# Simencassiman/P2PMicrogrid

Measured on AMD Instinct MI355X. Metric: agent-steps/sec (whole node, rollout+Q-update) at 1/2/4/8 MI355X; % HBM roofline, higher is better.
Workload: dtype f32 simulation, f64 Q-table

## Files before the change

### p2pmicrogrid_amd/csrc/p2pmg_fast.hip

```cpp
#include "p2pmg_fastmath.h"

namespace p2pmg {
namespace {

template <typename QT>
__device__ __forceinline__ Row4<QT> fake_row(const QT* p) {
  const uint32_t x = (uint32_t)(reinterpret_cast<uintptr_t>(p) >> 5);
  return Row4<QT>{{(QT)(x & 3), (QT)((x >> 2) & 3), (QT)((x >> 4) & 3), (QT)0}};
}

template <int N, int D, int G>
__device__ __forceinline__ void gather_even(float ev, float (&col)[N], int i) {
  if constexpr (D < G) {
    const float got = shfl_xor_c<D>(ev);
    const int src = i ^ D;
#pragma unroll
    for (int k = 0; k < N; ++k) col[k] = (k == src) ? got : col[k];
    gather_even<N, D + 1, G>(ev, col, i);
  }
}

#ifndef P2PMG_BAT_SPEC
#define P2PMG_BAT_SPEC 1
#endif
template <int N, typename QT, int R1, bool TRAIN, int BAT, bool NARROW, bool PIPE = false>
__global__ __launch_bounds__(kWave) void episode_fast_kernel(const EpisodeParams p, const uint2* __restrict__ pre,
                                                             FastRec* __restrict__ recs, int spw, int n_cons,
                                                             const PrepOut nxt) {
  if ((int)blockIdx.x >= n_cons) {
    const size_t n = (size_t)p.T * p.A, stride = (size_t)(gridDim.x - n_cons) * kWave;
    const int n_ep = nxt.n_ep > 1 ? nxt.n_ep : 1;
    for (int ep = 0; ep < n_ep; ++ep)
      for (size_t k2 = (size_t)(blockIdx.x - n_cons) * kWave + threadIdx.x; k2 < n; k2 += stride)
        prepass_one(p, nxt, k2, ep);
    return;
  }
  constexpr int G = pow2ceil(N);
  static_assert(G <= 8 && R1 >= 1 && R1 <= 4, "fast path: G <= 8, R + 1 <= 4");
  static_assert(!PIPE || (TRAIN && BAT == 0), "two episodes per wave: chained training launches without a battery");
  constexpr bool CAND = N == 2 && R1 >= 2 && BAT == 0;
  const int lane = (int)threadIdx.x;
  const int grp = PIPE ? lane >> 5 : 0;
  const int hl = PIPE ? (lane & 31) : lane;
  const int sl = hl / G;
  const int i = hl % G;
  const int s = (int)blockIdx.x * spw + sl;
  const bool active = i < N && sl < spw && s < p.S;
  const int a = active ? s * N + i : 0;
  const int s_env = p.n_env == 1 ? 0 : (active ? s : 0);
  const int T = p.T;
  const size_t A = (size_t)p.A;
  const KC k = pin_constants(p, p.thermal[a]);
  const uint32_t n_states = (uint32_t)(p.nt * p.nT * p.nb * p.np);
  QT* __restrict__ q = reinterpret_cast<QT*>(p.q) + (size_t)a * n_states * kQPad;
  const int a_first = (int)blockIdx.x * spw * N;
  constexpr uint32_t kRowShift = sizeof(QT) == 8 ? 5 : 4;
  const char* const qwave = reinterpret_cast<const char*>(p.q) + ((size_t)a_first * n_states << kRowShift);
  const uint32_t qlane = active ? (uint32_t)(a - a_first) * (n_states << kRowShift) : 0u;
  auto gat = [&](uint32_t row) __attribute__((always_inline)) {
    return gather_row(reinterpret_cast<const QT*>(qwave + (qlane + (row << kRowShift))));
  };
  const int np = k.np;
  const int nbv = k.nb;
  const float km1_T = (float)(k.nT - 1), km2_T = (float)(k.nT - 2), km1_p = (float)(np - 1), kp = (float)np;
  const float mi = active ? p.max_in[a] : 1.0f;
  const Recip rmi = recip(mi), rmph = recip(k.mph), rn = recip((float)N);
  const float4 lv = p.hp_lv[a];
  const float hin[3] = {(k.c_in * lv.x) * k.cop, (k.c_in * lv.y) * k.cop, (k.c_in * lv.z) * k.cop};
  const float hm[3] = {(k.c_m * lv.x) * k.cop, (k.c_m * lv.y) * k.cop, (k.c_m * lv.z) * k.cop};
  float tin = active ? p.t_in[a] : k.setpoint;
  float tm = active ? p.t_m[a] : k.setpoint;
  double bcap = 0.0, soc = 0.0;
  BatK bk{};
  Recip64 rcap{};
  if constexpr (BAT != 0) {
    bcap = active ? p.bat_cap[a] : 0.0;
    soc = active ? p.soc[a] : 0.0;
    bk = BatK{p.bat_min, p.bat_max, p.bat_sqrt_eff, recip64_u(p.bat_sqrt_eff), kR900};
    rcap = recip64(bcap > 0.0 ? bcap : 1.0);
  }
  const int ip_zero = idx_plain(div_n<N>(0.0f) / mi, np);
  QT* const q_dummy = reinterpret_cast<QT*>(p.dummy) + lane * kQPad;
  constexpr bool narrow = NARROW;
  const size_t rec_bytes = narrow ? sizeof(float2) : sizeof(FastRec);
  char* const rec_dummy = reinterpret_cast<char*>(reinterpret_cast<FastRec*>(p.dummy) + kWave + lane);
  const bool rec_on = p.record != 0 && active;
  const size_t rec_step = rec_on ? A * rec_bytes : 0;

  auto temp_bin = [&](float t_in) {
    const float x = t_in - k.setpoint;
    return clamp_bin_f(((x + 1.0f) / 2.0f) * km2_T + 1.0f, km1_T);
  };
  auto p2p_bin = [&](float x) { return clamp_bin_f(((x + 1.0f) / 2.0f) * kp, km1_p); };

  const float* envb = p.env + (size_t)s_env * kEnvStride;
  const size_t env_step = (size_t)p.n_env * kEnvStride;
  const uint2* preb = pre + a;
  const uint32_t* ipc_a = p.pre_ipc + a;
  const int t1 = T > 1 ? 1 : 0, t2 = 2 % T;
  const int n_chain = p.chain > 1 ? p.chain : 1;
  bool st_on = active;
  size_t rec_adv = rec_step;
  bool wrap_l = false;
  bool wrap_it = false;
  QT* snap = nullptr;
  if constexpr (PIPE) {
    __shared__ QT snap_lds[2 * 32 * 32];
    snap = snap_lds;
  }
  const uint32_t* codes_a;
  char* rec_ptr;
  uint32_t TA, env_st, env_end, o3, eo3;
  EnvV eS[3];
  uint2 pS[3];
  uint32_t cS[3];
  uint32_t cw, strip, a0, aN;
  int iT;
  Row4<QT> row0, rowN;
  uint32_t iS[3] = {0u, 0u, 0u};
  Row4<QT> cand[3];
  Patch<QT> pat{0xFFFFFFFFu, 0, (QT)0};
  float ep_sum = 0.0f;
  float t0_in = tin, t0_m = tm;
  auto code_of = [&](uint32_t w) { return TRAIN ? w : 0xFFFFFFFFu; };
  auto strip_of = [&](uint32_t base, int it_) { return __umul24(base + __umul24((uint32_t)it_, (uint32_t)nbv), (uint32_t)np); };
  auto row0_addr = [&](uint32_t st, uint32_t nr, uint32_t c) -> uint32_t {
    const bool need = ((c & 0xFF) == 255) || (TRAIN && R1 == 1);
    return need ? st + (uint32_t)ip_zero : nr;
  };
#if P2PMG_TRACE
  uint64_t trW = 0, trC = 0, trR = 0, trLast = 0, trA0 = 0, trWC = 0, trA1 = 0, trMid = 0, trCal = 0;
#define P2PMG_STAMP(v) asm volatile("s_memtime %0\n s_waitcnt lgkmcnt(0)" : "=s"(v)::"memory")
#endif
  auto begin_episode = [&](int ep) __attribute__((always_inline)) {
    if constexpr (PIPE) {
      if (ep >= 1 && st_on) {
        tin = t0_in;
        tm = t0_m;
      }
    }
    codes_a = p.codes + (size_t)(PIPE && ep < 0 ? 0 : ep) * p.codes_stride + a;
    if constexpr (PIPE) {
      rec_ptr = rec_on && st_on ? reinterpret_cast<char*>(recs) + (size_t)a * rec_bytes : rec_dummy;
      rec_adv = st_on ? rec_step : 0;
    } else {
      rec_ptr = rec_on ? reinterpret_cast<char*>(recs) + (size_t)a * rec_bytes : rec_dummy;
    }
    TA = (uint32_t)T * (uint32_t)A, env_st = (uint32_t)env_step, env_end = env_st * (uint32_t)T;
    o3 = (uint32_t)(3 % T) * (uint32_t)A, eo3 = (uint32_t)(3 % T) * env_st;

    eS[0] = load_envv(envb), eS[1] = load_envv(envb + (size_t)t1 * env_step), eS[2] = load_envv(envb + (size_t)t2 * env_step);
    pS[0] = preb[0], pS[1] = preb[(size_t)t1 * A], pS[2] = preb[(size_t)t2 * A];
    cS[0] = codes_a[0], cS[1] = codes_a[(size_t)t1 * A], cS[2] = codes_a[(size_t)t2 * A];
    cw = code_of(cS[0]);
    iT = temp_bin(tin);
    strip = strip_of(pS[0].y & 0xFFFFu, iT);
    const uint32_t nrow = strip_of(pS[0].y >> 16, iT) + (uint32_t)ip_zero;
    a0 = row0_addr(strip, nrow, cw);
    aN = TRAIN ? nrow : a0;
    row0 = gat(a0);
    rowN = gat(aN);
    if constexpr (CAND) {
      iS[0] = ipc_a[0];
      iS[1] = ipc_a[(size_t)t1 * A];
      iS[2] = ipc_a[(size_t)t2 * A];
#pragma unroll
      for (int b = 0; b < 3; ++b) cand[b] = gat((strip + ((iS[0] >> (8 * b)) & 0xFFu)));
    }
    pat = Patch<QT>{0xFFFFFFFFu, 0, (QT)0};
    ep_sum = 0.0f;
    if constexpr (!PIPE) {
      t0_in = tin, t0_m = tm;
      if (p.reset_t0 && active)
        t0_draw(p.seed_lo, p.seed_hi, p.episode + ep + 1, p.agent_offset + (uint32_t)a, k.setpoint, p.reset_sigma, t0_in,
                t0_m);
    } else {
      constexpr int kSnap = 10;
      const uint32_t key0 = pS[0].y & 0xFFFFu;
      const int nTi = p.nT;
      Row4<QT> sr[kSnap];
      auto snap_load = [&](int it0) {
#pragma unroll
        for (int j = 0; j < kSnap; ++j) sr[j] = gat(strip_of(key0, it0 + j < nTi ? it0 + j : nTi - 1) + (uint32_t)ip_zero);
      };
      auto snap_store = [&](int it0) {
#pragma unroll
        for (int j = 0; j < kSnap; ++j)
          if (it0 + j < nTi) snap[(grp * 32 + it0 + j) * 32 + hl] = max3(sr[j]);
      };
      snap_load(0);
      if (active)
        t0_draw(p.seed_lo, p.seed_hi, p.episode + (ep + 2 < n_chain ? ep + 2 : n_chain), p.agent_offset + (uint32_t)a,
                k.setpoint, p.reset_sigma, t0_in, t0_m);
      snap_store(0);
      for (int it0 = kSnap; it0 < nTi; it0 += kSnap) {
        snap_load(it0);
        snap_store(it0);
      }
    }
  };
  auto end_episode = [&](int ep) __attribute__((always_inline)) {
    if (active) {
      if (p.reset_t0) {
        tin = t0_in;
        tm = t0_m;
      }
      if (i == 0) {
        if (p.chain_rewards) p.chain_rewards[(size_t)ep * p.S + s] = ep_sum;
        if (ep == n_chain - 1) p.ep_reward[s] = ep_sum;
      }
    }
  };

  auto step = [&](auto par) __attribute__((always_inline)) {
    constexpr int P = decltype(par)::value, P1 = (P + 1) % 3;
    const EnvV ev = eS[P];
    const EnvRow e0{0.0f, ev.x, ev.y, ev.z, ev.w};
    const uint2 p0 = pS[P], p1 = pS[P1];
    const uint32_t c1 = cS[P1], ipc0 = iS[P], ipc1 = iS[P1];
    const float balw = __uint_as_float(p0.x);
    float row[N];
    float col[N];
#pragma unroll
    for (int j = 0; j < N; ++j) { row[j] = 0.0f; col[j] = 0.0f; }
    float tinA[3];
    uint32_t iTA[3], stA[3], nrA[3];
    {
      const float ain = k.inv_ri * (tm - tin) + k.inv_rvent * (e0.t_out - tin);
#pragma unroll
      for (int x = 0; x < 3; ++x) {
        const float d_in = k.inv_ci * (ain + hin[x]);
        tinA[x] = tin + (d_in * k.spm) * k.slot;
        iTA[x] = (uint32_t)temp_bin(tinA[x]);
        stA[x] = strip_of(p1.y & 0xFFFFu, (int)iTA[x]);
        nrA[x] = strip_of(p1.y >> 16, (int)iTA[x]) + (uint32_t)ip_zero;
      }
    }
    const Patch<QT> pprev = pat;
#if P2PMG_TRACE
    uint64_t tr0, tr1;
    P2PMG_STAMP(tr0);
    if (trLast) trR += tr0 - trLast;
    asm volatile("" ::"v"(row0.v[0]), "v"(row0.v[1]), "v"(row0.v[2]));
    P2PMG_STAMP(tr1);
    trW += tr1 - tr0;
    {
      uint64_t tcal;
      P2PMG_STAMP(tcal);
      trCal += tcal - tr1;
      tr1 = tcal;
    }
    trMid = tr1;
#endif
    double soc_r = soc;
    BatPre bpre{};
    if constexpr (BAT == 2) bpre = bat_pre(soc, bcap, bk);
    auto bat_rule = [&](float o, double& sr) -> float {
      if constexpr (BAT == 2) return (float)battery_rule_pre((double)o, sr, rcap, bk, bpre);
      return (float)battery_rule_r<true>((double)o, sr, bcap, rcap, bk);
    };
    row0 = patched(row0, a0, pat);

    int code = (int)(cw & 0xFF);
    int act = code == 255 ? argmax3(row0) : code;
    float hp = hp_of(lv, act);
    int ip = ip_zero;
    Row4<QT> rowR = row0;
    uint32_t acts = (uint32_t)act, ips = (uint32_t)ip_zero;
    float tin1 = tin, tm1 = tm;
    int iT1 = 0;
    uint32_t strip1 = 0, cw1 = 0, a0n = 0, aNn = 0;
    Row4<QT> row0n, rowNn, candn[3];
    Sel3M mnext{};
    auto issue_next = [&](int act_final) {
      const Sel3M m = sel3_masks(act_final);
// ... 117 lines not shown
        trC += trLast - trMid;
#endif
        refill_words();
        settle_next();
      }
      float out = balw + hp;
      if constexpr (BAT != 0) {
#if P2PMG_BAT_SPEC
        if (r == R1 - 1) {
          const Sel3M m = sel3_masks(act);
          out = sel3(m, outA[0], outA[1], outA[2]);
          soc_r = sel3(m, socA[0], socA[1], socA[2]);
        } else
#endif
        {
          soc_r = soc;
          if (bcap > 0.0) out = bat_rule(out, soc_r);
        }
      }
#if P2PMG_ABLATE == 11
      if (r == R1 - 1) {
        row[0] = out;
        continue;
      }
#endif
      const float flo = out < 0.0f ? 0.0f : -__builtin_inff(), fhi = out > 0.0f ? 0.0f : __builtin_inff();
      float f[N];
      float tot = 0.0f;
#pragma unroll
      for (int j = 0; j < N; ++j) {
        const float pw = -((j == i) ? 0.0f : col[j]);
        f[j] = __builtin_amdgcn_fmed3f(pw, flo, fhi);
        tot = tot + f[j];
      }
      tot = fabsf(tot);
      const float ev = div_n_r<N>(out * 1.0f, rn);
      const Recip rt = recip(tot == 0.0f ? 1.0f : tot);
      const float nout = nabs_out(out);
      float num[N];
      bool bad = !rt.ok;
#pragma unroll
      for (int j = 0; j < N; ++j) {
        num[j] = nout * f[j];
        row[j] = fdiv_core(num[j], rt);
        bad = bad || !fdiv_ok(num[j]);
      }
      if (bad) {
#pragma unroll
        for (int j = 0; j < N; ++j) row[j] = fdiv_ieee(num[j], rt.b);
      }
#pragma unroll
      for (int j = 0; j < N; ++j) row[j] = (tot == 0.0f) ? ev : row[j];
    }
    soc = soc_r;
    pat.row = 0xFFFFFFFFu;

    float g = 0.0f, pp = 0.0f;
#if P2PMG_ABLATE == 11
    g = row[0];
#else
    exchange<N>(row, col, i, sl, nullptr);
#pragma unroll
    for (int j = 0; j < N; ++j) {
      const float pij = row[j], pji = col[j];
      const float ex = pair_exchange(pij, pji);
      g = g + (pij - ex);
      pp = pp + ex;
    }
#endif
    float cost = (g >= 0.0f) ? g * e0.buy : g * e0.inj;
    cost = cost + pp * e0.p2p;
    cost = fdiv_b(cost * k.slot, rmph);
    cost = cost * k.kilo;
    float pen = fmaxf(fmaxf(0.0f, k.lower - tin), fmaxf(0.0f, tin - k.upper));
    pen = pen > 0.0f ? pen + 1.0f : 0.0f;
    const float rw = -(cost + k.penw * pen);

    if constexpr (TRAIN) {
      const uint32_t srow = strip + (uint32_t)ip;
      const QT qsa = sel3(act, rowR.v[0], rowR.v[1], rowR.v[2]);
      QT qmax = max3(patched(rowN, aN, pprev));
      if constexpr (PIPE && P == 2) {
        if (wrap_it) {
          const QT sv = snap[((grp ^ 1) * 32 + iT) * 32 + hl];
#if P2PMG_ABLATE != 12
          qmax = wrap_l ? sv : qmax;
#endif
        }
      }
      const QT qnew = td_update(qsa, rw, qmax, k.alpha, k.gamma);
      *((PIPE ? st_on : active) ? q + srow * kQPad + act : q_dummy) = qnew;
#if P2PMG_ABLATE == 9 || P2PMG_ABLATE == 10
      pat = Patch<QT>{0xFFFFFFFFu, 0, (QT)0};
#else
      pat = Patch<QT>{srow, act, qnew};
#endif
    }
    if constexpr (narrow) {
      *reinterpret_cast<float2*>(__builtin_assume_aligned(rec_ptr, 8)) = make_float2(rw, cost);
    } else {
      const uint32_t bins = (p0.y & 0xFFFFu) | ((uint32_t)iT << 16);
      float4* rp = reinterpret_cast<float4*>(__builtin_assume_aligned(rec_ptr, 16));
      rp[0] = make_float4(rw, cost, g, pp);
      rp[1] = make_float4(tin, __uint_as_float(acts), __uint_as_float(bins), __uint_as_float(ips));
    }
    rec_ptr += PIPE ? rec_adv : rec_step;
    asm volatile("" ::: "memory");
    eS[P] = load_envv(envb + eo3);
    pS[P] = preb[o3];
    const float m = group_sum<N>(rw, lane, i, sl, nullptr);
    ep_sum = ep_sum + div_n_r<N>(m, rn);

    tin = tin1;
    tm = tm1;
    iT = iT1;
    o3 += (uint32_t)A;
    o3 = o3 == TA ? 0u : o3;
    eo3 += env_st;
    eo3 = eo3 == env_end ? 0u : eo3;
    strip = strip1;
    cw = cw1;
    a0 = a0n;
    aN = aNn;
    row0 = row0n;
    rowN = rowNn;
    if constexpr (CAND) {
#pragma unroll
      for (int b = 0; b < 3; ++b) cand[b] = candn[b];
    }
  };
  using S0 = std::integral_constant<int, 0>;
  using S1 = std::integral_constant<int, 1>;
  using S2 = std::integral_constant<int, 2>;
  if constexpr (!PIPE) {
    for (int ep = 0; ep < n_chain; ++ep) {
      begin_episode(ep);
      __builtin_amdgcn_s_waitcnt(0);
      int t = 0;
      for (; t + 3 <= T; t += 3) {
        step(S0{});
        step(S1{});
        step(S2{});
      }
      if (t < T) step(S0{});
      if (t + 1 < T) step(S1{});
#if P2PMG_TRACE
      if (threadIdx.x == 0 && (blockIdx.x == 0 || (int)blockIdx.x == n_cons / 2 || (int)blockIdx.x == n_cons - 1))
        printf("TRACE blk %d/%d T %d: per step wait %.1f round0 %.1f waitcand %.1f round1 %.1f issue %.1f rest %.1f "
               "(one stamp %.1f)\n",
               (int)blockIdx.x, n_cons, T, (double)trW / T, (double)trA0 / T, (double)trWC / T, (double)trA1 / T,
               (double)trC / T, (double)trR / (T - 1), (double)trCal / T);
      trW = trC = trR = trLast = trA0 = trWC = trA1 = trMid = trCal = 0;
#endif
      end_episode(ep);
    }
    if (active) {
      p.t_in[a] = tin;
      p.t_m[a] = tm;
      if constexpr (BAT != 0) p.soc[a] = soc;
    }
  } else {
    const int L = T / 2;
    int ep_l = grp == 0 ? 0 : -1;
    st_on = active && grp == 0;
    begin_episode(ep_l);
    __builtin_amdgcn_s_waitcnt(0);
    for (int ph = 0;; ++ph) {
      if (ph > 0) {
        if (grp == (ph & 1)) {
          if (st_on && i == 0) {
            if (p.chain_rewards) p.chain_rewards[(size_t)ep_l * p.S + s] = ep_sum;
            if (ep_l == n_chain - 1) p.ep_reward[s] = ep_sum;
          }
          if (ph <= n_chain) {
            ep_l = ph;
            st_on = active && ph < n_chain;
            begin_episode(ph < n_chain ? ph : n_chain - 1);
          }
        }
        __builtin_amdgcn_s_waitcnt(0);
        if (ph > n_chain) break;
      }
      wrap_l = st_on && grp != (ph & 1) && ep_l + 1 < n_chain;
      for (int t = 0; t < L; t += 3) {
        wrap_it = t + 3 >= L;
        step(S0{});
        step(S1{});
        step(S2{});
      }
    }
    if (active && grp == ((n_chain - 1) & 1)) {
      p.t_in[a] = t0_in;
      p.t_m[a] = t0_m;
    }
  }
}

template <int N>
constexpr bool kFastPipe = N == 2;

template <int N, typename QT, int R1, int BAT, bool NARROW>
void launch_fast_nw(const EpisodeParams& p, const uint2* pre, FastRec* recs, int blocks, int spw, int prod,
                    const PrepOut& nxt, hipEvent_t ev0, hipEvent_t ev1, hipStream_t st) {
  if constexpr (kFastPipe<N> && BAT == 0) {
    if (p.mode == 0 && p.interleave)
      return hipExtLaunchKernelGGL((episode_fast_kernel<N, QT, R1, true, BAT, NARROW, true>), dim3(blocks + prod),
                                   dim3(kWave), 0, st, ev0, ev1, 0, p, pre, recs, spw, blocks, nxt);
  }
  if (p.mode == 0)
    hipExtLaunchKernelGGL((episode_fast_kernel<N, QT, R1, true, BAT, NARROW>), dim3(blocks + prod), dim3(kWave), 0, st,
                          ev0, ev1, 0, p, pre, recs, spw, blocks, nxt);
  else
    hipExtLaunchKernelGGL((episode_fast_kernel<N, QT, R1, false, BAT, NARROW>), dim3(blocks + prod), dim3(kWave), 0, st,
                          ev0, ev1, 0, p, pre, recs, spw, blocks, nxt);
}
template <int N, typename QT, int R1, int BAT>
void launch_fast_b(const EpisodeParams& p, const uint2* pre, FastRec* recs, int blocks, int spw, int prod,
                   const PrepOut& nxt, hipEvent_t ev0, hipEvent_t ev1, hipStream_t st) {
  if (p.rec_narrow) return launch_fast_nw<N, QT, R1, BAT, true>(p, pre, recs, blocks, spw, prod, nxt, ev0, ev1, st);
  launch_fast_nw<N, QT, R1, BAT, false>(p, pre, recs, blocks, spw, prod, nxt, ev0, ev1, st);
}
template <int N, typename QT, int R1>
void launch_fast_r(const EpisodeParams& p, const uint2* pre, FastRec* recs, int blocks, int spw, int prod,
                   const PrepOut& nxt, hipEvent_t ev0, hipEvent_t ev1, hipStream_t st) {
  if constexpr (R1 <= kFastBatMaxR1) {
    if (p.battery && p.bat_safe) return launch_fast_b<N, QT, R1, 2>(p, pre, recs, blocks, spw, prod, nxt, ev0, ev1, st);
    if (p.battery) return launch_fast_b<N, QT, R1, 1>(p, pre, recs, blocks, spw, prod, nxt, ev0, ev1, st);
  }
  launch_fast_b<N, QT, R1, 0>(p, pre, recs, blocks, spw, prod, nxt, ev0, ev1, st);
}

template <int N, typename QT>
hipError_t launch_fast_n(const EpisodeParams& p, const uint2* pre, void* recs, int spw, const PrepOut* nxt,
                         hipEvent_t ev0, hipEvent_t ev1, hipStream_t st) {
  constexpr int G = pow2ceil(N);
  if (p.interleave && !(kFastPipe<N> && p.mode == 0 && !p.battery && p.chain >= 2 && p.reset_t0 && p.T % 6 == 0 &&
                        p.nT <= 32 && spw > 0 && spw <= kWave / 2 / G))
    return hipErrorInvalidValue;
  if (spw <= 0 || spw > kWave / G) spw = kWave / G;
  const int blocks = (p.S + spw - 1) / spw;
  const size_t n = (size_t)p.T * p.A;
  const int prod = nxt ? (int)std::min<size_t>(2048, (n + kWave - 1) / kWave) : 0;
  const PrepOut none{nullptr, nullptr, nullptr, 0, 0.0};
  FastRec* r = reinterpret_cast<FastRec*>(recs);
  switch (p.R + 1) {
    case 1: launch_fast_r<N, QT, 1>(p, pre, r, blocks, spw, prod, nxt ? *nxt : none, ev0, ev1, st); break;
    case 2: launch_fast_r<N, QT, 2>(p, pre, r, blocks, spw, prod, nxt ? *nxt : none, ev0, ev1, st); break;
    case 3: launch_fast_r<N, QT, 3>(p, pre, r, blocks, spw, prod, nxt ? *nxt : none, ev0, ev1, st); break;
    case 4: launch_fast_r<N, QT, 4>(p, pre, r, blocks, spw, prod, nxt ? *nxt : none, ev0, ev1, st); break;
    default: return hipErrorInvalidValue;
  }
  return hipGetLastError();
}

template <int N0>
hipError_t launch_fast_pair(const EpisodeParams& p, const uint2* pre, void* recs, int q_dtype, int spw,
                            const PrepOut* nxt, hipEvent_t ev0, hipEvent_t ev1, hipStream_t st) {
  if (p.N == N0)
    return q_dtype == 0 ? launch_fast_n<N0, double>(p, pre, recs, spw, nxt, ev0, ev1, st)
                        : launch_fast_n<N0, float>(p, pre, recs, spw, nxt, ev0, ev1, st);
  if (p.N == N0 + 1)
    return q_dtype == 0 ? launch_fast_n<N0 + 1, double>(p, pre, recs, spw, nxt, ev0, ev1, st)
                        : launch_fast_n<N0 + 1, float>(p, pre, recs, spw, nxt, ev0, ev1, st);
  return hipErrorInvalidValue;
}

}

#define P2PMG_FAST_LAUNCHER(name, N0)                                                                             \
  hipError_t name(const EpisodeParams& p, const uint2* pre, void* recs, int q_dtype, int spw, const PrepOut* next, \
                  hipEvent_t ev0, hipEvent_t ev1, hipStream_t stream) {                                           \
    return launch_fast_pair<N0>(p, pre, recs, q_dtype, spw, next, ev0, ev1, stream);                              \
  }
#if P2PMG_FAST_SLICE == 0
P2PMG_FAST_LAUNCHER(launch_fast_n12, 1)
#endif
#if P2PMG_FAST_SLICE == 1
P2PMG_FAST_LAUNCHER(launch_fast_n34, 3)
#endif
#if P2PMG_FAST_SLICE == 2
P2PMG_FAST_LAUNCHER(launch_fast_n56, 5)
#endif
#if P2PMG_FAST_SLICE == 3
P2PMG_FAST_LAUNCHER(launch_fast_n78, 7)
#endif
#if P2PMG_FAST_SLICE == 0
hipError_t launch_episode_fast(const EpisodeParams& p, const uint2* pre, void* recs, int q_dtype, int spw,
                               const PrepOut* next, hipEvent_t ev0, hipEvent_t ev1, hipStream_t stream) {
  auto f = p.N <= 2 ? launch_fast_n12 : p.N <= 4 ? launch_fast_n34 : p.N <= 6 ? launch_fast_n56 : launch_fast_n78;
  if (p.N < 1 || p.N > 8) return hipErrorInvalidValue;
  return f(p, pre, recs, q_dtype, spw, next, ev0, ev1, stream);
}
#endif

}
```

### p2pmicrogrid_amd/csrc/p2pmg_plan.cpp

```cpp
#include "p2pmg_plan.h"

#include <algorithm>
#include <cmath>

#include "p2pmg_internal.h"

namespace p2pmg {
namespace {

bool host_div_range(float b) {
  const float m = std::fabs(b);
  return m >= 0x1p-40f && m <= 0x1p40f;
}

bool fast_applies(const PlanFacts& c, const p2pmg_episode_args& args, const Overrides& ov) {
  const p2pmg_config& g = c.cfg;
  return !g.shared_q && (!c.battery || c.R + 1 <= kFastBatMaxR1) && c.N <= 8 && c.R + 1 <= 4 && c.mi_ok &&
         (long long)g.n_time_states * g.n_temp_states * g.n_balance_states < 65536 &&
         64LL * g.n_time_states * g.n_temp_states * g.n_balance_states * g.n_p2p_states * 4 * (g.q_dtype == 0 ? 8 : 4) <
             (1LL << 32) &&
         (long long)c.T * c.A < (1LL << 32) && host_div_range(g.minutes_per_hour) &&
         g.temp_margin == 1.0f &&
         !(args.flags & (P2PMG_FLAG_GENERAL_KERNEL | P2PMG_FLAG_TILE_KERNEL | P2PMG_FLAG_PHILOX_INKERNEL)) &&
         !ov.general;
}

}

EpisodePlan plan_episode(const PlanFacts& c, const p2pmg_episode_args& args, bool chained, const Overrides& ov,
                         int n_chain) {
  const p2pmg_config& g = c.cfg;
  const bool train = args.mode == P2PMG_MODE_TRAIN;
  const bool philox = train && args.rng == P2PMG_RNG_PHILOX;
  const bool fast = fast_applies(c, args, ov);
  EpisodePlan pl;
  if (chained && !(fast && philox)) {
    pl.error = "run_episode: a chained launch needs the fast kernel and Philox training";
    return pl;
  }
  const bool sq16 = g.shared_q && !c.roles && c.N == 16 && c.R <= 1 && c.mi_ok && host_div_range(g.minutes_per_hour) &&
                    (long long)c.T * c.A < (1LL << 32) && (long long)c.T * c.n_env * kEnvStride < (1LL << 32) &&
                    host_div_range(g.temp_margin) && g.n_time_states == 20 && g.n_temp_states == 20 &&
                    g.n_balance_states == 20 && g.n_p2p_states == 20 &&
                    !c.thermal_set &&
                    !(args.flags & (P2PMG_FLAG_GENERAL_KERNEL | P2PMG_FLAG_TILE_KERNEL)) && !ov.general;
  const bool tile = !fast && !sq16 &&
                    ((args.flags & P2PMG_FLAG_TILE_KERNEL) != 0 || !((c.N >= 1 && c.N <= 8) || c.N == 16));
  pl.family = fast ? Family::Fast : sq16 ? Family::Sq16 : tile ? Family::Tile : Family::General;
  if (fast) {
    pl.philox = philox ? Philox::FastPrepass : Philox::None;
  } else if (philox) {
    bool prepass = c.A < (1 << 18) && !sq16;
    if (args.flags & P2PMG_FLAG_PHILOX_PREPASS) prepass = true;
    if (args.flags & P2PMG_FLAG_PHILOX_INKERNEL) prepass = false;
    pl.philox = prepass ? Philox::CodesPrepass : Philox::InKernel;
  }
  pl.want_ipc = fast && c.N == 2 && c.R >= 1 && !c.battery;
  pl.packed_records = fast || sq16;
  pl.rec_narrow = (fast || sq16) && (args.record & ~(P2PMG_REC_REWARD | P2PMG_REC_COST)) == 0 ? 1 : 0;
  pl.speculate = fast && !ov.no_spec;
  pl.interleave = fast && chained && n_chain >= 2 && philox && (args.flags & P2PMG_FLAG_RESET_T0) != 0 && !c.battery &&
                  c.T % 6 == 0 && g.n_temp_states <= 32 && c.N == 2 && c.chain_lag_ok && !ov.no_interleave;
  int spw = args.scen_per_wave > 0 ? args.scen_per_wave : ov.spw;
  if (spw <= 0) {
    const int full = 64 / (c.N <= 1 ? 1 : c.N <= 2 ? 2 : c.N <= 4 ? 4 : 8);
    const int waves = (c.S + full - 1) / full;
    spw = waves >= c.n_cu ? full : std::max(full / 4, (c.S + c.n_cu - 1) / c.n_cu);
    if (fast && train && args.epsilon < 0.5 && waves < c.n_cu) spw = std::max(full / 4, (spw + 1) / 2);
    spw = std::min(spw, full);
  }
  if (pl.interleave) spw = std::min(spw, 32 / 2);
  pl.spw = spw;
  return pl;
}

}
```

### p2pmicrogrid_amd/csrc/p2pmg_plan.h

```cpp
#pragma once
#include "p2pmg.h"

namespace p2pmg {

struct PlanFacts {
  p2pmg_config cfg{};
  int S = 0, N = 0, R = 0, T = 0, A = 0;
  int n_cu = 256;
  int n_env = 0;
  bool mi_ok = false;
  bool battery = false;
  bool roles = false;
  bool thermal_set = false;
  bool chain_lag_ok = false;
};

struct Overrides {
  bool general = false;
  int spw = 0;
  bool no_spec = false;
  bool no_interleave = false;
};

enum class Family { General, Tile, Fast, Sq16 };
enum class Philox { None, CodesPrepass, InKernel, FastPrepass };

struct EpisodePlan {
  Family family = Family::General;
  Philox philox = Philox::None;
  bool want_ipc = false;
  int spw = 0;
  int rec_narrow = 0;
  bool packed_records = false;
  bool speculate = false;
  bool interleave = false;
  const char* error = nullptr;
};

EpisodePlan plan_episode(const PlanFacts& c, const p2pmg_episode_args& args, bool chained, const Overrides& ov,
                         int n_chain = 1);

}
```

### p2pmicrogrid_amd/csrc/p2pmg_runtime.cpp

```cpp
#include "p2pmg.h"

#include <dlfcn.h>
#include <hip/hip_runtime.h>

#include <algorithm>
#include <climits>
#include <cmath>
#include <cstdint>
#include <cstdio>
#include <cstdlib>
#include <cstring>
#include <new>
#include <string>
#include <vector>

#include "p2pmg_internal.h"
#include "p2pmg_plan.h"

using p2pmg::EpisodeParams;
using p2pmg::EpisodePlan;
using p2pmg::Family;
using p2pmg::kEnvStride;
using p2pmg::kQPad;

// ... 26 lines not shown

 private:
  T* p_ = nullptr;
  size_t cap_ = 0;
};
template <typename T>
using PinBuf = DevBuf<T, true>;

struct EventRing {
  std::vector<hipEvent_t> ev;
  ~EventRing() {
    for (auto& e : ev)
      if (e) (void)hipEventDestroy(e);
  }
  hipError_t ensure(int slots) {
    if (!ev.empty()) return hipSuccess;
    ev.assign(2 * (size_t)slots, nullptr);
    for (auto& e : ev) {
      const hipError_t rc = hipEventCreate(&e);
      if (rc != hipSuccess) return rc;
    }
    return hipSuccess;
  }
  hipEvent_t* pair(long long k) { return &ev[2 * (size_t)(k % (long long)(ev.size() / 2))]; }
  hipError_t elapsed(long long k, float* ms) {
    const hipError_t e = hipEventSynchronize(pair(k)[1]);
    return e != hipSuccess ? e : hipEventElapsedTime(ms, pair(k)[0], pair(k)[1]);
  }
};

struct Stream {
  hipStream_t s = nullptr;
  ~Stream() {
    if (s) (void)hipStreamDestroy(s);
  }
  operator hipStream_t() const { return s; }
};

struct LastLaunch {
  int mask = 0;
  int packed_mask = 0;
  int narrow = 0;
  bool timed = false;
  std::string kernel;
};

struct p2pmg_ctx : p2pmg::PlanFacts {
  int device = 0;
  size_t n_states = 0;
  size_t q_elem = 8;
  Stream stream;
  static constexpr int kRing = 4096;
  EventRing ring;
  long long n_timed = 0;
  static constexpr int kCRing = 1024;
  EventRing cring;
  long long n_coll = 0;
  double coll_folded_ms = 0.0;
  long long n_coll_folded = 0;
  int timing_period = 1;
  long long n_launch = 0;
  LastLaunch last;
  DevBuf<float> env;
  DevBuf<float2> prof;
  DevBuf<uint2> sqp;
  long long sqp_version = -1;
  DevBuf<float> max_in, t_in, t_m;
  DevBuf<char> q;
  DevBuf<uint32_t> codes;
  DevBuf<uint2> pre[2];
  DevBuf<uint32_t> pre_ipc[2];
  DevBuf<uint32_t> pcodes[2];
  int pslot = 0;
  bool spec_valid[2] = {false, false};
  int spec_episode[2] = {0, 0};
  std::vector<double> spec_chain[2];
  DevBuf<float> chain_rew;
  int chain_n = 0;
  PinBuf<char> h_small;
  long long spec_version[2] = {-1, -1};
  long long inputs_version = 0;
  long long spec_hits = 0, spec_misses = 0;
  DevBuf<int> d_lag;
  int chain_lag = -1;
  long long lag_version = -1;
  DevBuf<char> dummy;
  DevBuf<char> rec_pack;
  int code_src = 0;
  DevBuf<float> ep_reward;
  DevBuf<float> rec_f32[5];
  DevBuf<uint8_t> rec_action;
  DevBuf<int32_t> rec_index;
  DevBuf<char> rec_stage;
  DevBuf<double> sum_agent, sum_scen;
  DevBuf<float4> hp_lv;
  DevBuf<float4> thermal;
  DevBuf<float> hp_on;
  DevBuf<double> soc, bat_cap;
  bool bat_domain = false;
  bool prof_bounded = false;
  bool hp_bounded = true;
  double bat_min = 0.1, bat_max = 0.9, bat_sqrt_eff = 1.0;
  size_t n_tables = 0;
  DevBuf<long long> qdelta;
  size_t delta_n() const { return n_tables * n_states * kQPad; }
  void* comm = nullptr;
  int rank = 0, nranks = 1;
  p2pmg_exchange_fn xfn = nullptr;
  void* xuser = nullptr;
  DevBuf<double> d_metrics;
  DevBuf<unsigned long long> d_hash;
  bool have_env = false, have_prof = false, have_params = false, have_codes = false;
  bool dqn = false;
  p2pmg_dqn_config dcfg{};
  int n_nets = 0;
  DevBuf<float> d_theta, d_target, d_m, d_v;
  DevBuf<float> d_grad;
  DevBuf<float> d_alt;
  DevBuf<float> d_segs;
  PinBuf<float> h_segs;
  DevBuf<float> d_smp;
  int d_blocks = 0, d_apb = 1;
  int d_seg_local = 1, d_seg_agents = 0, d_bps = 0;
  DevBuf<float> d_buf;
  DevBuf<int32_t> d_added;
  DevBuf<uint16_t> d_samples;
  DevBuf<uint16_t> d_samples_px;
  bool have_samples = false;
  DevBuf<float> d_ep_acc;
  DevBuf<float> rec_loss;
  std::vector<int64_t> d_steps;
  DevBuf<float> d_lr;
  std::vector<float> h_lr;
  int64_t d_added_min = 0;
  std::string err;
};

struct Id128 {
  char b[128];
};
struct Rccl {
  void* h = nullptr;
  int (*getUniqueId)(void*) = nullptr;
  int (*commInitRank)(void**, int, Id128, int) = nullptr;
  int (*allReduce)(const void*, void*, size_t, int, int, void*, hipStream_t) = nullptr;
  int (*commDestroy)(void*) = nullptr;
  const char* (*getErrorString)(int) = nullptr;
  int (*allGather)(const void*, void*, size_t, int, void*, hipStream_t) = nullptr;
  int (*commCount)(const void*, int*) = nullptr;
};
static Rccl* rccl() {
  static Rccl r;
  static bool tried = false;
  if (!tried) {
    tried = true;
    const char* names[] = {"librccl.so.1", "librccl.so", "/opt/rocm/lib/librccl.so.1"};
    for (const char* n : names) {
      r.h = dlopen(n, RTLD_NOW | RTLD_GLOBAL);
      if (r.h) break;
    }
    if (r.h) {
      r.getUniqueId = (int (*)(void*))dlsym(r.h, "ncclGetUniqueId");
      r.commInitRank = (int (*)(void**, int, Id128, int))dlsym(r.h, "ncclCommInitRank");
      r.allReduce = (int (*)(const void*, void*, size_t, int, int, void*, hipStream_t))dlsym(r.h, "ncclAllReduce");
      r.commDestroy = (int (*)(void*))dlsym(r.h, "ncclCommDestroy");
      r.getErrorString = (const char* (*)(int))dlsym(r.h, "ncclGetErrorString");
      r.allGather = (int (*)(const void*, void*, size_t, int, void*, hipStream_t))dlsym(r.h, "ncclAllGather");
      r.commCount = (int (*)(const void*, int*))dlsym(r.h, "ncclCommCount");
    }
  }
  return (r.h && r.getUniqueId && r.commInitRank && r.allReduce && r.commDestroy) ? &r : nullptr;
}

namespace {

int fail(p2pmg_ctx* c, int code, const std::string& msg) {
  if (c) c->err = msg;
  return code;
}

#define HIP_TRY(ctx, expr)                                                                       \
  do {                                                                                           \
    hipError_t _e = (expr);                                                                      \
    if (_e != hipSuccess)                                                                        \
      return fail((ctx), _e == hipErrorOutOfMemory ? P2PMG_E_NOMEM : P2PMG_E_HIP,                \
                  std::string(#expr) + ": " + hipGetErrorString(_e));                            \
  } while (0)

#define RC_TRY(expr)                      \
  do {                                    \
    const int _rc = (expr);               \
    if (_rc != P2PMG_OK) return _rc;      \
  } while (0)

int rec_slot(int which) {
  switch (which) {
    case P2PMG_REC_REWARD: return 0;
    case P2PMG_REC_COST: return 1;
    case P2PMG_REC_GRID: return 2;
    case P2PMG_REC_P2P: return 3;
    case P2PMG_REC_TEMP: return 4;
    default: return -1;
  }
}

int ensure_records(p2pmg_ctx* c, int mask) {
  const size_t ta = (size_t)c->T * c->A;
  for (int b = 0; b < 5; ++b)
    if ((mask & (1 << b)) && !c->rec_f32[b]) HIP_TRY(c, c->rec_f32[b].alloc(ta));
  const size_t tra = (size_t)c->T * (c->R + 1) * c->A;
  if ((mask & P2PMG_REC_ACTION) && !c->rec_action) HIP_TRY(c, c->rec_action.alloc(tra));
  if ((mask & P2PMG_REC_INDEX) && !c->rec_index) HIP_TRY(c, c->rec_index.alloc(tra));
  if ((mask & P2PMG_REC_LOSS) && !c->rec_loss) HIP_TRY(c, c->rec_loss.alloc(ta));
  return P2PMG_OK;
}

const p2pmg::Overrides& overrides() {
  static const p2pmg::Overrides ov = [] {
    const char *k = getenv("P2PMG_KERNEL"), *w = getenv("P2PMG_SPW"), *n = getenv("P2PMG_NO_SPEC");
    const char* il = getenv("P2PMG_INTERLEAVE");
    return p2pmg::Overrides{k && !strcmp(k, "general"), w ? atoi(w) : 0, n && atoi(n) != 0, il && atoi(il) == 0};
  }();
  return ov;
}

struct Timed {
  hipEvent_t e0 = nullptr, e1 = nullptr;
};

int begin_timed(p2pmg_ctx* c, bool sampled, bool record, Timed* t) {
  HIP_TRY(c, c->ring.ensure(p2pmg_ctx::kRing));
  if (sampled && (c->n_launch++ % c->timing_period) != 0) return P2PMG_OK;
  t->e0 = c->ring.pair(c->n_timed)[0];
  t->e1 = c->ring.pair(c->n_timed)[1];
  if (record) HIP_TRY(c, hipEventRecord(t->e0, c->stream));
  return P2PMG_OK;
}

int end_timed(p2pmg_ctx* c, const Timed& t, bool record) {
  if (record && t.e1) HIP_TRY(c, hipEventRecord(t.e1, c->stream));
  return P2PMG_OK;
}

void finish_launch(p2pmg_ctx* c, const Timed& t, std::string kernel, int mask, int packed_mask, int narrow) {
  c->last.kernel = std::move(kernel);
  c->last.mask = mask;
  c->last.packed_mask = packed_mask;
  c->last.narrow = narrow;
  c->last.timed = true;
  if (t.e1) c->n_timed++;
}

}

extern "C" {

int p2pmg_abi_version(void) { return P2PMG_ABI_VERSION; }

int p2pmg_device_count(int* count) {
  if (!count) return P2PMG_E_INVALID;
  int n = 0;
  if (hipGetDeviceCount(&n) != hipSuccess) n = 0;
  *count = n;
  return P2PMG_OK;
}

int p2pmg_config_default(p2pmg_config* cfg) {
  if (!cfg) return P2PMG_E_INVALID;
  std::memset(cfg, 0, sizeof(*cfg));
  cfg->n_scenarios = 1;
  cfg->n_agents = 2;
  cfg->rounds = 1;
  cfg->horizon = 96;
  cfg->q_dtype = P2PMG_Q_F64;
  cfg->n_time_states = cfg->n_temp_states = cfg->n_balance_states = cfg->n_p2p_states = 20;
  cfg->n_actions = 3;
  cfg->alpha = 1e-5;
  cfg->gamma = 0.9;
  const double levels[3] = {0.0, 0.5, 1.0};
  for (int k = 0; k < 3; ++k) cfg->hp_levels[k] = (float)(levels[k] * 3e3);
  cfg->setpoint = 21.0f;
  cfg->temp_margin = 1.0f;
  cfg->lower_bound = 20.0f;
  cfg->upper_bound = 22.0f;
  const double Ci = 2.44e6 * 2, Cm = 9.4e7, Ri = 8.64e-4, Re = 1.05e-2, Rvent = 7.98e-3, gA = 11.468, f_rad = 0.3;
  cfg->inv_ci = (float)(1 / Ci);
  cfg->inv_cm = (float)(1 / Cm);
  cfg->inv_ri = (float)(1 / Ri);
  cfg->inv_re = (float)(1 / Re);
  cfg->inv_rvent = (float)(1 / Rvent);
  cfg->one_minus_frad = (float)(1 - f_rad);
  cfg->frad = (float)f_rad;
  cfg->solar_gain = (float)(gA * 0.0);
  cfg->hp_cop = 3.0f;
  cfg->seconds_per_minute = 60.0f;
  cfg->time_slot = 15.0f;
  cfg->minutes_per_hour = 60.0f;
  cfg->kilo = (float)1e-3;
  cfg->penalty_weight = 10.0f;
  cfg->seed = 42;
  cfg->scenario_offset = 0;
  return P2PMG_OK;
}

// ... 399 lines not shown
    for (int k = 0; k < o.n_ep; ++k) {
      int all = 0;
      p2pmg::eps_threshold(eps[k], o.ep_thr[k], all);
      o.ep_all |= (uint64_t)all << k;
    }
    return o;
  };
  const bool hit = c->spec_valid[ps] && c->spec_version[ps] == c->inputs_version &&
                   (!philox || (c->spec_episode[ps] == args->episode && c->spec_chain[ps] == cur));
  if (!hit) HIP_TRY(c, p2pmg::launch_step_prepass(p, prep_out(ps, args->episode, cur), c->stream));
  const int ns = ps ^ 1;
  *next = prep_out(ns, args->episode + n_ep, nxt_eps);
  if (hit) c->spec_hits++;
  else c->spec_misses++;
  c->spec_valid[ns] = plan.speculate;
  c->spec_version[ns] = c->inputs_version;
  c->spec_episode[ns] = philox ? args->episode + n_ep : -1;
  c->spec_chain[ns] = nxt_eps;
  return P2PMG_OK;
}

static int prepare_sq16(p2pmg_ctx* c, const p2pmg_episode_args* args, EpisodeParams& p) {
  RC_TRY(ensure_rec_pack(c, args));
  p.rec_pack = c->rec_pack;
  if (!c->sqp) HIP_TRY(c, c->sqp.alloc((size_t)c->T * c->A));
  if (c->sqp_version != c->inputs_version) {
    HIP_TRY(c, p2pmg::launch_sq16_prep(p, c->sqp, c->stream));
    c->sqp_version = c->inputs_version;
  }
  p.sqp = c->sqp;
  return P2PMG_OK;
}

static int prepare_general(p2pmg_ctx* c, const p2pmg_episode_args* args, const EpisodePlan& plan, EpisodeParams& p) {
  RC_TRY(ensure_records(c, args->record));
  bind_records(c, p);
  if (plan.philox != p2pmg::Philox::CodesPrepass) return P2PMG_OK;
  RC_TRY(ensure_codes(c));
  p.codes = c->codes;
  HIP_TRY(c, p2pmg::launch_philox_codes(p, c->codes, c->stream));
  c->code_src = 2;
  c->have_codes = false;
  p.rng = 0;
  return P2PMG_OK;
}

static int update_chain_lag(p2pmg_ctx* c, const uint2* pre) {
  if (c->lag_version == c->inputs_version) return P2PMG_OK;
  c->chain_lag = -1;
  if (c->T <= p2pmg::kChainLagMaxT) {
    if (!c->d_lag) HIP_TRY(c, c->d_lag.alloc(1));
    HIP_TRY(c, p2pmg::launch_chain_lag(c->T, c->A, pre, c->d_lag, c->stream));
    HIP_TRY(c, hipMemcpyAsync(&c->chain_lag, c->d_lag, sizeof(int), hipMemcpyDeviceToHost, c->stream));
    HIP_TRY(c, hipStreamSynchronize(c->stream));
  }
  c->chain_lag_ok = c->chain_lag >= 0 && c->chain_lag + 4 <= c->T / 2;
  c->lag_version = c->inputs_version;
  return P2PMG_OK;
}

static int run_episode_impl(p2pmg_ctx* c, const p2pmg_episode_args* args, const ChainReq* ch) {
  if (!c || !args) return P2PMG_E_INVALID;
  if (c->dqn) return dqn_run_episode(c, args);
  if (!c->have_env || !c->have_prof || !c->have_params)
    return fail(c, P2PMG_E_STATE, "run_episode: env, profiles and agent params must be set first");
  const bool train = args->mode == P2PMG_MODE_TRAIN;
  if (args->mode != P2PMG_MODE_TRAIN && args->mode != P2PMG_MODE_GREEDY) return fail(c, P2PMG_E_INVALID, "mode");
  if (train && args->rng != P2PMG_RNG_REPLAY && args->rng != P2PMG_RNG_PHILOX) return fail(c, P2PMG_E_INVALID, "rng");
  if (train && args->rng == P2PMG_RNG_REPLAY && !c->have_codes)
    return fail(c, P2PMG_E_STATE, "run_episode: replay mode needs p2pmg_set_replay_codes");
  EpisodePlan plan = p2pmg::plan_episode(*c, *args, ch != nullptr, overrides(), ch ? ch->n : 1);
  if (plan.error) return fail(c, P2PMG_E_INVALID, plan.error);
  const p2pmg_config& g = c->cfg;
  const bool fast = plan.family == Family::Fast, sq16 = plan.family == Family::Sq16, tile = plan.family == Family::Tile;
  const bool ext = plan.packed_records;
  EpisodeParams p = episode_params(c, args);
  const int ps = c->pslot;
  p2pmg::PrepOut next{};
  RC_TRY(fast ? prepare_fast(c, args, ch, plan, p, &next) : sq16 ? prepare_sq16(c, args, p) : prepare_general(c, args, plan, p));
  if (fast && ch && c->lag_version != c->inputs_version) {
    RC_TRY(update_chain_lag(c, c->pre[ps]));
    plan = p2pmg::plan_episode(*c, *args, true, overrides(), ch->n);
  }
  p.interleave = plan.interleave ? 1 : 0;
  p.rec_narrow = plan.rec_narrow;
  const bool reset = (args->flags & P2PMG_FLAG_RESET_T0) != 0;
  p.reset_t0 = (ext && reset) ? 1 : 0;
  p.reset_sigma = args->reset_sigma;
  Timed tm;
  RC_TRY(begin_timed(c, true, !ext, &tm));
  hipError_t e = fast   ? p2pmg::launch_episode_fast(p, c->pre[ps], c->rec_pack, g.q_dtype, plan.spw,
                                                    plan.speculate ? &next : nullptr, tm.e0, tm.e1, c->stream)
                 : sq16 ? p2pmg::launch_episode_sq16(p, g.q_dtype, tm.e0, tm.e1, c->stream)
                        : p2pmg::launch_episode(p, g.q_dtype, tile, c->stream);
  if (e != hipSuccess) return fail(c, P2PMG_E_HIP, std::string("episode launch: ") + hipGetErrorString(e));
  RC_TRY(end_timed(c, tm, !ext));
  if (fast) c->pslot ^= 1;
  if (reset && !ext) {
    const uint32_t off = (uint32_t)(g.scenario_offset * c->N);
    HIP_TRY(c, p2pmg::launch_t0_philox(c->A, c->t_in, c->t_m, p.seed_lo, p.seed_hi, args->episode + 1, off,
                                       c->thermal, args->reset_sigma, c->stream));
  }
  finish_launch(c, tm,
                std::string(fast ? "episode_fast_kernel<" : sq16 ? "episode_sq16_kernel<" : "episode_kernel<") +
                    std::to_string(c->N) + (tile ? ",tile" + std::to_string(p2pmg::general_tile_cap(c->N)) : "") + "," +
                    (g.q_dtype == 0 ? "f64" : "f32") + ",R1=" + std::to_string(c->R + 1) +
                    (ext ? (train ? ",train" : ",greedy") : "") + (g.shared_q ? ",shared" : "") + (c->roles ? ",roles" : "") +
                    (c->battery ? (ext && !p.bat_safe ? ",battery,range-checked>" : ",battery>")
                                : plan.interleave ? ",interleaved>" : ">"),
                args->record, ext ? (args->record & 127) : 0, plan.rec_narrow);
  return P2PMG_OK;
}

int p2pmg_run_episodes(p2pmg_ctx* c, const p2pmg_episode_args* args, int n, const double* epsilons, int next_n,
                       const double* next_epsilons) {
  if (!c || !args || n < 1 || !epsilons || (next_n > 0 && !next_epsilons)) return P2PMG_E_INVALID;
  if (!c->dqn && (!c->have_env || !c->have_prof || !c->have_params))
    return fail(c, P2PMG_E_STATE, "run_episodes: env, profiles and agent params must be set first");
  HIP_TRY(c, c->chain_rew.grow((size_t)std::max(n, p2pmg::kMaxChain) * c->S));
  c->chain_n = 0;
  const bool chain = !c->dqn && p2pmg::plan_episode(*c, *args, false, overrides()).philox == p2pmg::Philox::FastPrepass;
  p2pmg_episode_args a = *args;
  if (!chain) {
    for (int k = 0; k < n; ++k) {
      a.episode = args->episode + k;
      a.epsilon = epsilons[k];
      a.flags = args->flags | P2PMG_FLAG_NEXT_EPSILON;
      a.next_epsilon = k + 1 < n ? epsilons[k + 1] : next_n > 0 ? next_epsilons[0] : epsilons[k];
      RC_TRY(run_episode_impl(c, &a, nullptr));
      HIP_TRY(c, hipMemcpyAsync(c->chain_rew + (size_t)k * c->S, c->ep_reward,
                                (size_t)c->S * sizeof(float), hipMemcpyDeviceToDevice, c->stream));
    }
    c->chain_n = n;
    return P2PMG_OK;
  }
  const size_t wpe_bytes = (size_t)c->T * c->A * ((c->R + 4) / 4) * sizeof(uint32_t);
  const int per = (int)std::max<size_t>(1, std::min<size_t>(p2pmg::kMaxChain, ((size_t)1 << 30) / wpe_bytes));
  for (int k0 = 0; k0 < n; k0 += per) {
    const int m = std::min(per, n - k0);
    const int k1 = k0 + m;
    ChainReq req{m, epsilons + k0, 0, nullptr, c->chain_rew + (size_t)k0 * c->S, per};
    if (k1 < n) {
      req.next_n = std::min(per, n - k1);
      req.next_eps = epsilons + k1;
    } else if (next_n > 0) {
      req.next_n = std::min(per, next_n);
      req.next_eps = next_epsilons;
    }
    a.episode = args->episode + k0;
    a.epsilon = epsilons[k0];
    RC_TRY(run_episode_impl(c, &a, &req));
  }
  c->chain_n = n;
  return P2PMG_OK;
}

int p2pmg_get_episode_rewards(p2pmg_ctx* c, int n, float* host) {
  if (!c || !host || n < 0) return P2PMG_E_INVALID;
  if (n > c->chain_n) return fail(c, P2PMG_E_STATE, "get_episode_rewards: the last run_episodes call ran fewer episodes");
  HIP_TRY(c, hipMemcpyAsync(host, c->chain_rew, (size_t)n * c->S * sizeof(float), hipMemcpyDeviceToHost, c->stream));
  HIP_TRY(c, hipStreamSynchronize(c->stream));
  return P2PMG_OK;
}

int p2pmg_chain_lag(p2pmg_ctx* c, int* distance, int* safe) {
  if (!c) return P2PMG_E_INVALID;
  if (c->lag_version != c->inputs_version)
    return fail(c, P2PMG_E_STATE, "chain_lag: no chained launch has run since the last input upload");
  if (distance) *distance = c->chain_lag;
  if (safe) *safe = c->chain_lag_ok ? 1 : 0;
  return P2PMG_OK;
}

int p2pmg_set_timing_period(p2pmg_ctx* c, int period) {
  if (!c || period < 1) return P2PMG_E_INVALID;
  c->timing_period = period;
  c->n_launch = 0;
  return P2PMG_OK;
}

static int ensure_hp_on(p2pmg_ctx* c) {
  if (c->hp_on) return P2PMG_OK;
  HIP_TRY(c, c->hp_on.alloc((size_t)c->A));
  HIP_TRY(c, hipMemsetAsync(c->hp_on, 0, (size_t)c->A * sizeof(float), c->stream));
  return P2PMG_OK;
}

int p2pmg_set_hp_state(p2pmg_ctx* c, const float* on) {
  if (!c || !on) return P2PMG_E_INVALID;
  RC_TRY(ensure_hp_on(c));
  HIP_TRY(c, hipMemcpyAsync(c->hp_on, on, (size_t)c->A * sizeof(float), hipMemcpyHostToDevice, c->stream));
  HIP_TRY(c, hipStreamSynchronize(c->stream));
// ... 1054 lines not shown
```

Measured before the change: 16.19 billion.

## Generalize episode interleaving to four chained episodes per wave

Replaces the fixed two-episodes-per-wave pipelined training kernel with a DEPTH template parameter, so a wavefront can run 2 or 4 staggered chained episodes in separate lane groups. The snapshot LDS, wrap-around Q max lookup, phase scheduling and t0 draw offsets are generalized to K groups. The planner picks depth 4 when T divides by 12 and the chain lag fits within a quarter episode, with a clamped scenarios-per-wave. The aim is to hide more of the serial per-step latency across episodes. The cost is fewer scenarios per lane group and more LDS per wave.

```diff
diff --git a/p2pmicrogrid_amd/csrc/p2pmg_fast.hip b/p2pmicrogrid_amd/csrc/p2pmg_fast.hip
--- a/p2pmicrogrid_amd/csrc/p2pmg_fast.hip
+++ b/p2pmicrogrid_amd/csrc/p2pmg_fast.hip
@@ -23,7 +23,7 @@
 #ifndef P2PMG_BAT_SPEC
 #define P2PMG_BAT_SPEC 1
 #endif
-template <int N, typename QT, int R1, bool TRAIN, int BAT, bool NARROW, bool PIPE = false>
+template <int N, typename QT, int R1, bool TRAIN, int BAT, bool NARROW, int DEPTH = 0>
 __global__ __launch_bounds__(kWave) void episode_fast_kernel(const EpisodeParams p, const uint2* __restrict__ pre,
                                                              FastRec* __restrict__ recs, int spw, int n_cons,
                                                              const PrepOut nxt) {
@@ -36,12 +36,16 @@
     return;
   }
   constexpr int G = pow2ceil(N);
+  constexpr bool PIPE = DEPTH != 0;
+  constexpr int K = PIPE ? DEPTH : 1;
+  constexpr int GL = kWave / K;
   static_assert(G <= 8 && R1 >= 1 && R1 <= 4, "fast path: G <= 8, R + 1 <= 4");
-  static_assert(!PIPE || (TRAIN && BAT == 0), "two episodes per wave: chained training launches without a battery");
+  static_assert(DEPTH == 0 || DEPTH == 2 || DEPTH == 4, "episodes per wave: 2 or 4");
+  static_assert(!PIPE || (TRAIN && BAT == 0), "several episodes per wave: chained training launches without a battery");
   constexpr bool CAND = N == 2 && R1 >= 2 && BAT == 0;
   const int lane = (int)threadIdx.x;
-  const int grp = PIPE ? lane >> 5 : 0;
-  const int hl = PIPE ? (lane & 31) : lane;
+  const int grp = PIPE ? lane / GL : 0;
+  const int hl = PIPE ? lane % GL : lane;
   const int sl = hl / G;
   const int i = hl % G;
   const int s = (int)blockIdx.x * spw + sl;
@@ -105,7 +109,7 @@
   bool wrap_it = false;
   QT* snap = nullptr;
   if constexpr (PIPE) {
-    __shared__ QT snap_lds[2 * 32 * 32];
+    __shared__ QT snap_lds[K * 32 * GL];
     snap = snap_lds;
   }
   const uint32_t* codes_a;
@@ -186,11 +190,11 @@
       auto snap_store = [&](int it0) {
 #pragma unroll
         for (int j = 0; j < kSnap; ++j)
-          if (it0 + j < nTi) snap[(grp * 32 + it0 + j) * 32 + hl] = max3(sr[j]);
+          if (it0 + j < nTi) snap[(grp * 32 + it0 + j) * GL + hl] = max3(sr[j]);
       };
       snap_load(0);
       if (active)
-        t0_draw(p.seed_lo, p.seed_hi, p.episode + (ep + 2 < n_chain ? ep + 2 : n_chain), p.agent_offset + (uint32_t)a,
+        t0_draw(p.seed_lo, p.seed_hi, p.episode + (ep + K < n_chain ? ep + K : n_chain), p.agent_offset + (uint32_t)a,
                 k.setpoint, p.reset_sigma, t0_in, t0_m);
       snap_store(0);
       for (int it0 = kSnap; it0 < nTi; it0 += kSnap) {
@@ -474,7 +478,7 @@
       QT qmax = max3(patched(rowN, aN, pprev));
       if constexpr (PIPE && P == 2) {
         if (wrap_it) {
-          const QT sv = snap[((grp ^ 1) * 32 + iT) * 32 + hl];
+          const QT sv = snap[(((grp + 1) % K) * 32 + iT) * GL + hl];
 #if P2PMG_ABLATE != 12
           qmax = wrap_l ? sv : qmax;
 #endif
@@ -552,28 +556,28 @@
       if constexpr (BAT != 0) p.soc[a] = soc;
     }
   } else {
-    const int L = T / 2;
-    int ep_l = grp == 0 ? 0 : -1;
+    const int L = T / K;
+    int ep_l = grp == 0 ? 0 : grp - K;
     st_on = active && grp == 0;
     begin_episode(ep_l);
     __builtin_amdgcn_s_waitcnt(0);
     for (int ph = 0;; ++ph) {
       if (ph > 0) {
-        if (grp == (ph & 1)) {
+        if (grp == ph % K) {
           if (st_on && i == 0) {
             if (p.chain_rewards) p.chain_rewards[(size_t)ep_l * p.S + s] = ep_sum;
             if (ep_l == n_chain - 1) p.ep_reward[s] = ep_sum;
           }
-          if (ph <= n_chain) {
+          if (ph < n_chain + K - 1) {
             ep_l = ph;
             st_on = active && ph < n_chain;
             begin_episode(ph < n_chain ? ph : n_chain - 1);
           }
         }
         __builtin_amdgcn_s_waitcnt(0);
-        if (ph > n_chain) break;
-      }
-      wrap_l = st_on && grp != (ph & 1) && ep_l + 1 < n_chain;
+        if (ph >= n_chain + K - 1) break;
+      }
+      wrap_l = st_on && ep_l + K - 1 == ph && ep_l + 1 < n_chain;
       for (int t = 0; t < L; t += 3) {
         wrap_it = t + 3 >= L;
         step(S0{});
@@ -581,7 +585,7 @@
         step(S2{});
       }
     }
-    if (active && grp == ((n_chain - 1) & 1)) {
+    if (active && grp == (n_chain - 1) % K) {
       p.t_in[a] = t0_in;
       p.t_m[a] = t0_m;
     }
@@ -595,8 +599,11 @@
 void launch_fast_nw(const EpisodeParams& p, const uint2* pre, FastRec* recs, int blocks, int spw, int prod,
                     const PrepOut& nxt, hipEvent_t ev0, hipEvent_t ev1, hipStream_t st) {
   if constexpr (kFastPipe<N> && BAT == 0) {
-    if (p.mode == 0 && p.interleave)
-      return hipExtLaunchKernelGGL((episode_fast_kernel<N, QT, R1, true, BAT, NARROW, true>), dim3(blocks + prod),
+    if (p.mode == 0 && p.interleave == 4)
+      return hipExtLaunchKernelGGL((episode_fast_kernel<N, QT, R1, true, BAT, NARROW, 4>), dim3(blocks + prod),
+                                   dim3(kWave), 0, st, ev0, ev1, 0, p, pre, recs, spw, blocks, nxt);
+    if (p.mode == 0 && p.interleave == 2)
+      return hipExtLaunchKernelGGL((episode_fast_kernel<N, QT, R1, true, BAT, NARROW, 2>), dim3(blocks + prod),
                                    dim3(kWave), 0, st, ev0, ev1, 0, p, pre, recs, spw, blocks, nxt);
   }
   if (p.mode == 0)
@@ -626,8 +633,9 @@
 hipError_t launch_fast_n(const EpisodeParams& p, const uint2* pre, void* recs, int spw, const PrepOut* nxt,
                          hipEvent_t ev0, hipEvent_t ev1, hipStream_t st) {
   constexpr int G = pow2ceil(N);
-  if (p.interleave && !(kFastPipe<N> && p.mode == 0 && !p.battery && p.chain >= 2 && p.reset_t0 && p.T % 6 == 0 &&
-                        p.nT <= 32 && spw > 0 && spw <= kWave / 2 / G))
+  if (p.interleave && !((p.interleave == 2 || p.interleave == 4) && kFastPipe<N> && p.mode == 0 && !p.battery &&
+                        p.chain >= 2 && p.reset_t0 && p.T % (3 * p.interleave) == 0 && p.nT <= 32 && spw > 0 &&
+                        spw <= kWave / p.interleave / G))
     return hipErrorInvalidValue;
   if (spw <= 0 || spw > kWave / G) spw = kWave / G;
   const int blocks = (p.S + spw - 1) / spw;
diff --git a/p2pmicrogrid_amd/csrc/p2pmg_plan.cpp b/p2pmicrogrid_amd/csrc/p2pmg_plan.cpp
--- a/p2pmicrogrid_amd/csrc/p2pmg_plan.cpp
+++ b/p2pmicrogrid_amd/csrc/p2pmg_plan.cpp
@@ -59,8 +59,13 @@
   pl.packed_records = fast || sq16;
   pl.rec_narrow = (fast || sq16) && (args.record & ~(P2PMG_REC_REWARD | P2PMG_REC_COST)) == 0 ? 1 : 0;
   pl.speculate = fast && !ov.no_spec;
-  pl.interleave = fast && chained && n_chain >= 2 && philox && (args.flags & P2PMG_FLAG_RESET_T0) != 0 && !c.battery &&
-                  c.T % 6 == 0 && g.n_temp_states <= 32 && c.N == 2 && c.chain_lag_ok && !ov.no_interleave;
+  const bool pipe = fast && chained && n_chain >= 2 && philox && (args.flags & P2PMG_FLAG_RESET_T0) != 0 && !c.battery &&
+                    g.n_temp_states <= 32 && c.N == 2 && c.chain_lag_ok && !ov.no_interleave;
+  if (pipe && ov.max_depth >= 4 && c.T % 12 == 0 && c.chain_lag >= 0 && c.chain_lag + 4 <= c.T / 4)
+    pl.depth = 4;
+  else if (pipe && c.T % 6 == 0)
+    pl.depth = 2;
+  pl.interleave = pl.depth != 0;
   int spw = args.scen_per_wave > 0 ? args.scen_per_wave : ov.spw;
   if (spw <= 0) {
     const int full = 64 / (c.N <= 1 ? 1 : c.N <= 2 ? 2 : c.N <= 4 ? 4 : 8);
@@ -69,7 +74,8 @@
     if (fast && train && args.epsilon < 0.5 && waves < c.n_cu) spw = std::max(full / 4, (spw + 1) / 2);
     spw = std::min(spw, full);
   }
-  if (pl.interleave) spw = std::min(spw, 32 / 2);
+  if (pl.depth == 2) spw = std::min(spw, 64 / 2 / 2);
+  if (pl.depth == 4) spw = std::min(std::max(spw, 32 / 4), 64 / 4 / 2);
   pl.spw = spw;
   return pl;
 }
diff --git a/p2pmicrogrid_amd/csrc/p2pmg_plan.h b/p2pmicrogrid_amd/csrc/p2pmg_plan.h
--- a/p2pmicrogrid_amd/csrc/p2pmg_plan.h
+++ b/p2pmicrogrid_amd/csrc/p2pmg_plan.h
@@ -13,6 +13,7 @@
   bool roles = false;
   bool thermal_set = false;
   bool chain_lag_ok = false;
+  int chain_lag = -1;
 };
 
 struct Overrides {
@@ -20,6 +21,7 @@
   int spw = 0;
   bool no_spec = false;
   bool no_interleave = false;
+  int max_depth = 4;
 };
 
 enum class Family { General, Tile, Fast, Sq16 };
@@ -34,6 +36,7 @@
   bool packed_records = false;
   bool speculate = false;
   bool interleave = false;
+  int depth = 0;
   const char* error = nullptr;
 };
 
diff --git a/p2pmicrogrid_amd/csrc/p2pmg_runtime.cpp b/p2pmicrogrid_amd/csrc/p2pmg_runtime.cpp
--- a/p2pmicrogrid_amd/csrc/p2pmg_runtime.cpp
+++ b/p2pmicrogrid_amd/csrc/p2pmg_runtime.cpp
@@ -132,7 +132,6 @@
   long long inputs_version = 0;
   long long spec_hits = 0, spec_misses = 0;
   DevBuf<int> d_lag;
-  int chain_lag = -1;
   long long lag_version = -1;
   DevBuf<char> dummy;
   DevBuf<char> rec_pack;
@@ -269,7 +268,8 @@
   static const p2pmg::Overrides ov = [] {
     const char *k = getenv("P2PMG_KERNEL"), *w = getenv("P2PMG_SPW"), *n = getenv("P2PMG_NO_SPEC");
     const char* il = getenv("P2PMG_INTERLEAVE");
-    return p2pmg::Overrides{k && !strcmp(k, "general"), w ? atoi(w) : 0, n && atoi(n) != 0, il && atoi(il) == 0};
+    return p2pmg::Overrides{k && !strcmp(k, "general"), w ? atoi(w) : 0, n && atoi(n) != 0, il && atoi(il) == 0,
+                            il && atoi(il) == 2 ? 2 : 4};
   }();
   return ov;
 }
@@ -835,7 +835,7 @@
     RC_TRY(update_chain_lag(c, c->pre[ps]));
     plan = p2pmg::plan_episode(*c, *args, true, overrides(), ch->n);
   }
-  p.interleave = plan.interleave ? 1 : 0;
+  p.interleave = plan.depth;
   p.rec_narrow = plan.rec_narrow;
   const bool reset = (args->flags & P2PMG_FLAG_RESET_T0) != 0;
   p.reset_t0 = (ext && reset) ? 1 : 0;
@@ -860,7 +860,7 @@
                     (g.q_dtype == 0 ? "f64" : "f32") + ",R1=" + std::to_string(c->R + 1) +
                     (ext ? (train ? ",train" : ",greedy") : "") + (g.shared_q ? ",shared" : "") + (c->roles ? ",roles" : "") +
                     (c->battery ? (ext && !p.bat_safe ? ",battery,range-checked>" : ",battery>")
-                                : plan.interleave ? ",interleaved>" : ">"),
+                                : plan.depth == 4 ? ",x4,interleaved>" : plan.interleave ? ",interleaved>" : ">"),
                 args->record, ext ? (args->record & 127) : 0, plan.rec_narrow);
   return P2PMG_OK;
 }
```

Result: no change. 16.34 billion, median of 6 (+0.9%).
